# calad0i/da4ml

Measured on AMD Instinct MI355X. Metric: CMVM solves/sec, 256x256 int8 matrix, higher is better.
Workload: dtype u32; 1 GPU; c3_256x256_int8_batch64_single_chain; matrix=256x256 int8 (default_rng(seed).integers(-128,128)), batch_per_gpu=64, parallelism=1 x independent-instance shard, no data-path collective

## Files before the change

### __graft_entry__.py

```python

import subprocess
import sys
from pathlib import Path

ROOT = Path(__file__).resolve().parent
if str(ROOT) not in sys.path:
    sys.path.insert(0, str(ROOT))


def build() -> None:
    subprocess.run(['make', '-C', str(ROOT / 'da4ml_amd' / 'csrc')], check=True)
    subprocess.run(['make', '-C', str(ROOT / 'oracle'), 'liboracle.so', 'ref'], check=True)
    subprocess.run(['make', '-C', str(ROOT / 'tests' / 'model')], check=True)
    subprocess.run(['make', '-C', str(ROOT / 'tests' / 'geometry')], check=True)
    subprocess.run(['make', '-C', str(ROOT / 'tests' / 'tie_order')], check=True)
    subprocess.run(['make', '-C', str(ROOT / 'tests' / 'dc_rank')], check=True)
    subprocess.run(['make', '-C', str(ROOT / 'tests' / 'emu')], check=True)
    import da4ml_amd
    from da4ml_amd import _binary

    lib = _binary.lib()
    missing = [s for s in _binary.EXPORTS if not hasattr(lib, s)]
    assert not missing, f'libda4ml_hip.so lacks {missing}'


def smoke() -> None:
    import numpy as np

    from da4ml_amd import _binary
# ... 16 lines not shown
```

### da4ml_amd/_binary/__init__.py

```python

from __future__ import annotations

import ctypes as C
from pathlib import Path
from types import SimpleNamespace

import numpy as np

from .._marshal import pipeline_from_stages, stage_from_arrays

import os as _os

_LIB_PATH = Path(_os.environ['DA4ML_HIP_LIB']).resolve() if _os.environ.get('DA4ML_HIP_LIB') else Path(__file__).resolve().parent.parent / 'libda4ml_hip.so'
_lib = None

_f32p = np.ctypeslib.ndpointer(np.float32, flags='C_CONTIGUOUS')
_i64p = np.ctypeslib.ndpointer(np.int64, flags='C_CONTIGUOUS')
_i32p = np.ctypeslib.ndpointer(np.int32, flags='C_CONTIGUOUS')

EXPORTS = (
    'da_last_error da_last_error_code da_version da_device_count da_set_device da_get_lsb_loc da_iceil_log2 da_cost_add da_int_arr_to_csd '
    'da_csd_decompose da_kernel_decompose da_solve da_solve_batch da_solve_batch_seeded da_solve_batch_opts da_solve_sharded da_rccl_unique_id da_rccl_shutdown da_solve_sharded_rccl da_comm_abort da_shard_exchanged_elements da_n_stages da_picked da_stage_info da_stage_copy '
    'da_result_stats da_free da_timings da_engine_stats da_dais_run da_dais_last_error da_dais_run_on'
).split()
# ... 425 lines not shown
        _raise(rc)
    return RawBatch([res[i] for i in range(n)])


def timings(reset: bool = False) -> dict:
    t = np.zeros(32, np.float64)
    e = np.zeros(16, np.float64)
    lib().da_engine_stats(e, 16)
    rc = lib().da_timings(t, int(reset))
    if rc != 0:
        _raise(rc)
    names = ('loop_ms', 'dist_ms', 'total_ms', 'lockstep_iters', 'iterations', 'rescans', 'partners', 'chains', 'table_bytes', 'arena_bytes',
             'select_ms_sampled', 'update_ms_sampled', 'samples', 'found', 'inserts', 'cell_reads', 'block_bytes', 'cell_bytes',
             'sel_load_bounds', 'sel_argmax', 'sel_newrow', 'sel_substitute', 'sel_prefix', 'sel_claims', 'sel_special',
             'upd_fetch', 'upd_probe', 'upd_cells', 'upd_blocks', 'upd_create', 'retries', 'sampled_chain_launches')
    extra = ('select_bytes', 'host_launch_ms', 'fast_steps', 'search_bounds', 'search_argmax', 'search_excluded', 'search_steps_timed', 'search_stale_rereads', 'search_touch_rereads', 'search_rounds', 'search_long_lists', 'search_longest_list', 'search_full_passes', 'search_list_entries', 'manycol_chains')
    return {**dict(zip(names, t.tolist())), **dict(zip(extra, e.tolist()))}


_DAIS_EXECUTORS = {'host': 0, 'cpu': 0, 'device': 1, 'gpu': 1, 'host-scalar': 2}


def dais_interp_run(bin_logic, data, n_threads: int = 1, executor: str = 'host'):
    prog = np.ascontiguousarray(np.ravel(bin_logic), dtype=np.int32)
    if prog.size < 4:
        raise RuntimeError('Invalid binary logic data')
    n_in, n_out = int(prog[2]), int(prog[3])
    x = np.ascontiguousarray(np.ravel(data), dtype=np.float64)
    assert n_in > 0 and x.size % n_in == 0, f'Input size {x.size} is not divisible by {n_in}'
    n_samples = x.size // n_in
    out = np.zeros((n_samples, max(n_out, 0)), dtype=np.float64)
# ... 17 lines not shown
```

### da4ml_amd/csrc/cmvm_capi.cc

```cpp

#include <cstdlib>
#include <chrono>
#include <cstdio>
#include <pthread.h>

#include <algorithm>
#include <atomic>
#include <limits>
#include <cstring>
#include <memory>
#include <mutex>
#include <new>
#include <string>
#include <vector>

#include "../../include/da4ml_hip.h"
#include "cmvm_gpu.h"
#include "cmvm_host.h"
#include "cmvm_rccl.h"
#include "cmvm_shard.h"

namespace {

thread_local std::string g_err;
// ... 385 lines not shown
        for (int q = 0; q < 12; ++q) v[18 + q] = g.phase_cycles[q];
        v[30] = (double)g.retries;
        v[31] = g.sampled_chain_launches;
        std::memcpy(t, v, sizeof v);
        if (reset) be.reset_timings();
        return DA_OK;
    } catch (const std::exception &e) {
        return fail(e);
    }
}

int da_engine_stats(double *out, int n) {
    std::lock_guard<LibraryMutex> lk(g_mutex);
    try {
        const da::gpu::GpuTimings &g = backend().timings();
        const double v[16] = {g.select_bytes, g.host_launch_ms, (double)g.fast_steps, g.search_cycles[0], g.search_cycles[1], g.search_cycles[2], g.search_cycles[3], g.search_diag[0], g.search_diag[1], g.search_diag[2], g.search_diag[3], g.search_diag[4], g.search_diag[5], g.search_diag[6], (double)g.manycol_chains, 0.0};
        const int m = n < 16 ? (n < 0 ? 0 : n) : 16;
        for (int i = 0; i < m; ++i) out[i] = v[i];
        return m;
    } catch (const std::exception &e) {
        fail(e);
        return 0;
    }
}

}
```

### da4ml_amd/csrc/cmvm_engine.hip

```cpp

#include <hip/hip_runtime.h>

#include <algorithm>
#include <atomic>
#include <chrono>
#include <cmath>
#include <cstdio>
#include <cstdlib>
#include <cstring>
#include <memory>
#include <mutex>
#include <numeric>
#include <stdexcept>
#include <string>
#include <thread>
#include <type_traits>
#include <vector>

#include "cmvm_core.h"
#include "cmvm_geometry.h"
#include "cmvm_gpu.h"
#include "cmvm_host.h"

namespace da {
// ... 241 lines not shown
    unsigned long long st_sel_bytes;
    unsigned long long st_phase[12];
    SpecPick spec[2];
    unsigned int c_n[2], l_n[2];
    CandEntry c_list[2][CAND_CAP];
    CandEntry l_list[2][TOUCH_CAP];
    uint32_t *sp_cnt;
    unsigned long long st_fast;
    unsigned long long st_qphase[4];
#ifdef DA_STEP_CLOCKS
    unsigned long long clk[2][4];
#endif
    unsigned long long st_qdiag[9];
    unsigned long long tie_seed;
    float dc_weight;
};

__constant__ Log2Table c_log2;

__device__ __forceinline__ int lane_id() { return threadIdx.x & (WAVE - 1); }
__device__ __forceinline__ int wave_id() { return threadIdx.x / WAVE; }

template <int CTRL, int ROW_MASK> __device__ __forceinline__ uint32_t dpp_u32(uint32_t identity, uint32_t v) {
    return (uint32_t)__builtin_amdgcn_update_dpp((int)identity, (int)v, CTRL, ROW_MASK, 0xF, false);
}
constexpr int DPP_ROW_SHR1 = 0x111, DPP_ROW_SHR2 = 0x112, DPP_ROW_SHR4 = 0x114, DPP_ROW_SHR8 = 0x118, DPP_ROW_BCAST15 = 0x142, DPP_ROW_BCAST31 = 0x143;
#define DA_DPP_REDUCE32(v, ident, OP)                                   \
    v = OP(v, dpp_u32<DPP_ROW_SHR1, 0xF>(ident, v));                    \
    v = OP(v, dpp_u32<DPP_ROW_SHR2, 0xF>(ident, v));                    \
    v = OP(v, dpp_u32<DPP_ROW_SHR4, 0xF>(ident, v));                    \
// ... 202 lines not shown
    } else {
        atomicMax(gen(&c.grec[grp].glow), w_old);
    }
}
__device__ __forceinline__ void fold_entry(const Ctx &c, uint32_t rank, unsigned long long tie) {
    if (c.rword && bound_word(rank, tie) >= c.rword) {
        const unsigned int at = atomicAdd(c.cn, 1u);
        if (at < (unsigned int)CAND_CAP) {
            c.cl[at].rank = rank;
            c.cl[at].tie = tie;
        }
    }
}
__device__ __forceinline__ DA_GLOBAL uint8_t *hidx_ptr(const Ctx &c) { return reinterpret_cast<DA_GLOBAL uint8_t *>(c.hrank + ((size_t)c.cmask + 1)); }

template <bool SEEDED, bool WEIGHTED>
__device__ __forceinline__ void publish_new_block(const BlockEval<SEEDED, WEIGHTED> &ev, int slot, uint32_t lo, uint32_t hi, int ov, float dl, unsigned long long best) {
    const Ctx &c = ev.c;
    const uint32_t rank = ev.rank_of_best(best), idx = ev.idx_of_best(best);
    store_hdr(c, slot, ov, dl, rank, idx);
    c.hrank[slot] = rank;
    hidx_ptr(c)[slot] = (uint8_t)idx;
    if (rank) {
        group_note(c, slot, 0ull, bound_word(rank, ev.tie(lo, hi, idx)));
        fold_entry(c, rank, ev.tie(lo, hi, idx));
    }
}

template <bool SEEDED, bool WEIGHTED, class CntFn>
__device__ bool table_insert(const BlockEval<SEEDED, WEIGHTED> &ev, uint32_t lo, uint32_t hi, const RowInfo &ra, const RowInfo &rb, CntFn cnt_of, bool tally = true) {
    const Ctx &c = ev.c;
    int lane = lane_id();
    unsigned long long key = pack_pair(lo, hi);
    int slot = table_claim(c, key, hash_pair(lo, hi));
    if (slot < 0) {
        if (lane == 0) c.g->error = E_TABLE_CAPACITY;
        return false;
// ... 12 lines not shown
    if (lane == 0) {
        publish_new_block(ev, slot, lo, hi, ov, dl, best);
        if (tally) atomicAdd(&c.g->n_live, 1u);
    }
    return true;
}

template <bool SEEDED, bool WEIGHTED>
__device__ __forceinline__ void block_commit(const BlockEval<SEEDED, WEIGHTED> &ev, int slot, unsigned long long key, const BlkHdr &h, unsigned long long best, int alive, bool tally = true) {
    const Ctx &c = ev.c;
    const uint32_t lo = (uint32_t)key, hi = (uint32_t)(key >> 32);
    const unsigned long long w_old = ev.word(lo, hi, h.rank, h.idx);
    if (!alive) {
        c.hrank[slot] = 0;
        c.hkey[slot] = c.tomb;
        if (tally) atomicSub(&c.g->n_live, 1u);
        if (h.rank) group_note(c, slot, w_old, 0ull);
        return;
    }
    const uint32_t rank = ev.rank_of_best(best), idx = ev.idx_of_best(best);
    if (rank != h.rank) c.hrank[slot] = rank;
    if (rank != h.rank || idx != h.idx) store_best(c, slot, rank, idx);
    if (idx != h.idx) hidx_ptr(c)[slot] = (uint8_t)idx;
    if (rank != h.rank || (rank && idx != h.idx)) group_note(c, slot, w_old, ev.word(lo, hi, rank, idx));
    if (rank) fold_entry(c, rank, ev.tie(lo, hi, idx));
}

template <bool SEEDED, bool WEIGHTED, class CntFn>
__device__ bool table_update(const BlockEval<SEEDED, WEIGHTED> &ev, int slot, unsigned long long key, CntFn new_cnt, bool tally = true) {
    const Ctx &c = ev.c;
// ... 108 lines not shown
}

__device__ __forceinline__ void fill16(void *p, size_t bytes, uint32_t v, size_t t0, size_t stride) {
    da_i4 *q = reinterpret_cast<da_i4 *>(p);
    const da_i4 w = da_i4{(int)v, (int)v, (int)v, (int)v};
    for (size_t i = t0, n = (bytes + 15) / 16; i < n; i += stride) q[i] = w;
}
__global__ void __launch_bounds__(256) k_init_state(ChainDev *chains) {
    const ChainDev &ch = chains[blockIdx.y];
    const size_t t0 = (size_t)blockIdx.x * blockDim.x + threadIdx.x, stride = (size_t)gridDim.x * blockDim.x;
    fill16(ch.stamp, sizeof(uint32_t) * (size_t)ch.rcap, 0u, t0, stride);
    fill16(ch.hkey, sizeof(unsigned long long) * (size_t)ch.C, 0xFFFFFFFFu, t0, stride);
    fill16(ch.hrank, sizeof(uint32_t) * (size_t)ch.C, 0u, t0, stride);
    for (size_t i = t0; i < (size_t)ch.n_groups; i += stride) ch.grec[i] = GroupRec{0ull, 0ull, 0ull, 1u, 0u};
    fill16(ch.colbits, sizeof(uint32_t) * (size_t)ch.n_out * ch.cb_words, 0u, t0, stride);
}

template <class Cell> __global__ void __launch_bounds__(256) k_init_cells(ChainDev *chains) {
    using O = CellOps<Cell>;
    using F = RowFmt<Cell>;
    ChainDev &ch = chains[blockIdx.y];
    int j = blockIdx.x * (blockDim.x / WAVE) + wave_id();
    if (j >= ch.n_out) return;
    auto *rl = reinterpret_cast<typename F::Entry *>(ch.rlist);
    int lane = lane_id(), len = 0;
    for (int base = 0; base < ch.n_in; base += WAVE) {
        int i = base + lane;
        Cell c = 0;
        if (i < ch.n_in) {
            bool dead = ch.qints[3 * i] == 0.0f && ch.qints[3 * i + 1] == 0.0f;
// ... 505 lines not shown
    float sp_rb0 = g->spec[par ^ 1].rb.lo, sp_rb1 = g->spec[par ^ 1].rb.hi, sp_rb2 = g->spec[par ^ 1].rb.step, sp_rb3 = g->spec[par ^ 1].rb.lat;
    Ctx c = make_ctx_raw<SEEDED>(g, 2 * iter);
    DA_GLOBAL int *collen = (DA_GLOBAL int *)g->collen;
    DA_GLOBAL da_u2 *rowoff = (DA_GLOBAL da_u2 *)g->rowoff;
    DA_GLOBAL Entry *rl = (DA_GLOBAL Entry *)g->rlist;
    DA_GLOBAL Cell *mA = (DA_GLOBAL Cell *)g->mA, *mB = (DA_GLOBAL Cell *)g->mB;
    DA_GLOBAL int *mcol = (DA_GLOBAL int *)g->mcol;
    DA_GLOBAL unsigned long long *collist = (DA_GLOBAL unsigned long long *)g->collist;
    DA_GLOBAL uint16_t *cmap = (DA_GLOBAL uint16_t *)g->cmap;
    DA_GLOBAL uint32_t *colbits = (DA_GLOBAL uint32_t *)g->colbits;
    DA_GLOBAL uint32_t *pl_ids = (DA_GLOBAL uint32_t *)g->pl_ids;
    DA_GLOBAL unsigned long long *plist = (DA_GLOBAL unsigned long long *)g->plist;
    DA_GLOBAL da_i4 *picks = (DA_GLOBAL da_i4 *)g->picks;
    DA_GLOBAL uint32_t *sp_cnt = (DA_GLOBAL uint32_t *)g->sp_cnt;
    DA_GLOBAL int32_t *cs_slab = (DA_GLOBAL int32_t *)g->cs_slab, *cs_flags = (DA_GLOBAL int32_t *)g->cs_flags;
    pin_sgpr(was_done, had_error, lcap, claim_words, n_rows0, rcap, cbw, adder_size, carry_size, offN, rl_cap, n_live0, live_peak0, step_mant, step_tab, n_step_mant);
    pin_sgpr(sp_word, sp_tie, cn_prev, cl_prev, sp_ax, sp_ay, sp_bx, sp_by, sp_ra0, sp_ra1, sp_ra2, sp_ra3, sp_rb0, sp_rb1, sp_rb2, sp_rb3);
    pin_sgpr(c.n_out, c.n_bits, c.K, c.Kpad, c.rows);
    pin_sgpr(collen, rowoff, rl, mA, mB, mcol, collist, cmap, colbits, pl_ids, plist, picks, sp_cnt);
    if constexpr (SHARDED) pin_sgpr(cs_slab, cs_flags);
    if constexpr (SEEDED) pin_sgpr(c.seed);
    const int n_out = c.n_out, Kpad = c.Kpad, nb = c.n_bits;
    auto shard_stop = [&](int err) {
        if constexpr (SHARDED) {
            const int fw = (n_rows0 + 3) / 4;
            for (int w = threadIdx.x; w < fw; w += SEL2_THREADS) cs_flags[w] = 0;
            if (threadIdx.x == 0) {
                const bool cap = err == E_ROW_CAPACITY || err == E_TABLE_CAPACITY || err == E_LIST_CAPACITY;
                cs_flags[fw] = 1;
                cs_flags[fw + 1] = cap ? 1 : 0;
                cs_flags[fw + 2] = err != E_OK && !cap ? 1 : 0;
            }
        }
    };
    if (was_done) {
        shard_stop(had_error);
// ... 8 lines not shown
    Idx *s_bpos = s_col + n_out;
    int *s_clen = reinterpret_cast<int *>(s_bpos + n_out);
    Idx *s_cm = reinterpret_cast<Idx *>(s_clen + n_out);
    uint32_t *s_or = reinterpret_cast<uint32_t *>(s_cm + n_out);
    if constexpr (MANYCOL) {
        s_bent = nullptr;
        s_clen = nullptr;
        s_cnt = reinterpret_cast<uint32_t *>(smem);
        s_len = reinterpret_cast<int *>(s_cnt + 6 * Kpad);
        s_or = reinterpret_cast<uint32_t *>(s_len + n_out + 1);
        s_col = reinterpret_cast<Idx *>(s_or + claim_words);
        s_bpos = s_col + n_out;
        s_cm = s_bpos + n_out;
    }
    constexpr int NW = SEL2_THREADS / WAVE;
    __shared__ int s_np, s_part[NW];
    __shared__ unsigned int s_matches;
    __shared__ RowInfo s_new;
    __shared__ unsigned long long s_am_tie[NW];
    __shared__ uint32_t s_am_rank[NW];
    constexpr int IDS_LDS = DA_IDS_LDS;
    __shared__ uint32_t s_ids[IDS_LDS];
    __shared__ Log2Table s_log2;

    const int tid = threadIdx.x, lane = lane_id(), wid = wave_id();

    SEL_TIMER_DECL
    SEL_TIMER_MARK(0)
    if (had_error != E_OK) {
        if (tid == 0) {
            g->done = 1;
// ... 11 lines not shown
    da_u2 refA = da_u2{sp_ax, sp_ay}, refB = da_u2{sp_bx, sp_by};
    RowInfo ra = RowInfo{sp_ra0, sp_ra1, sp_ra2, sp_ra3}, rb = RowInfo{sp_rb0, sp_rb1, sp_rb2, sp_rb3};
    if (fast && !from_spec) {
        refA = rowoff[A];
        refB = rowoff[B];
        ra = load_row(c.rows, A);
        rb = load_row(c.rows, B);
    }
    {
        int clen0 = 0;
        if constexpr (!MANYCOL) clen0 = collen[tid < n_out ? tid : 0];
        const bool want_log2 = (adder_size >= 0 || carry_size >= 0) && tid < (int)(sizeof(Log2Table) / 4);
        const uint32_t l2w = want_log2 ? reinterpret_cast<const uint32_t *>(&c_log2)[tid] : 0u;
        if (tid == 0) {
            s_np = 0;
            s_matches = 0;
            g->c_n[par] = 0;
        }
        if (tid < n_out) {
            if constexpr (!MANYCOL) s_clen[tid] = clen0;
            s_cm[tid] = 0;
            s_bpos[tid] = 0;
        }
        if (want_log2) reinterpret_cast<uint32_t *>(&s_log2)[tid] = l2w;
        for (int w = tid; w < claim_words; w += SEL2_THREADS) s_or[w] = 0;
        for (int j = tid + SEL2_THREADS; j < n_out; j += SEL2_THREADS) {
            if constexpr (!MANYCOL) s_clen[j] = collen[j];
            s_cm[j] = 0;
            s_bpos[j] = 0;
        }
// ... 41 lines not shown
        shard_stop(E_LIST_CAPACITY);
        return 1;
    }
    DA_GLOBAL Entry *rlA = rl + refA.x, *rlB = rl + refB.x, *rlN = rl + offN;
    Entry eA0 = rl[tid < lenA ? refA.x + (uint32_t)tid : 0u], eB0 = rl[tid < lenB ? refB.x + (uint32_t)tid : 0u];
    load_fence();
    RowInfo rn = RowInfo{0.0f, 0.0f, 0.0f, 0.0f};
    int derr = 0;
    if (tid == 0) {
        qint_add_pair(ra, rb, shift, sub, rn.lo, rn.hi, rn.step);
        float dlat = adder_dlat(ra, rb, shift, sub, adder_size, carry_size, s_log2, StepLog2{n_step_mant, step_mant, step_tab}, derr);
        rn.lat = (ra.lat < rb.lat ? rb.lat : ra.lat) + dlat;
        s_new = rn;
    }
    for (int k = tid; k < 6 * Kpad; k += SEL2_THREADS) s_cnt[k] = 0;
    if (tid >= lenA) eA0 = F::none();
    if (same || tid >= lenB) eB0 = F::none();
    pin_vgpr(eA0, eB0);
    if (!same) {
        if (tid < lenB) {
            if constexpr (!MANYCOL) s_bent[tid] = eB0;
            s_bpos[F::col(eB0)] = (Idx)(tid + 1);
        }
        for (int t = tid + SEL2_THREADS; t < lenB; t += SEL2_THREADS) {
            const Entry e = rlB[t];
            if constexpr (!MANYCOL) s_bent[t] = e;
            s_bpos[F::col(e)] = (Idx)(t + 1);
        }
    }
    if (tid == 0) {
// ... 105 lines not shown
    __syncthreads();
    SEL_TIMER_MARK(4)
    SEL_TIMER_MARK(5)
    if constexpr (SHARDED) {
        for (int k = tid; k < 6 * c.K; k += SEL2_THREADS) {
            const int sp = k / c.K;
            cs_slab[k] = (same && (sp == 1 || sp == 2 || sp == 4)) ? 0 : (int32_t)s_cnt[sp * Kpad + (k - sp * c.K)];
        }
    } else
        for (int k = tid; k < 6 * Kpad; k += SEL2_THREADS) sp_cnt[k] = s_cnt[k];
    {
        const DA_GLOBAL uint32_t *cb = colbits;
        const int nwords = (int)((Nw + 31) >> 5), chunks = (nwords + WAVE - 1) / WAVE;
        DA_GLOBAL uint32_t *ids = pl_ids;
        const bool split = chunks * 4 <= NW && m >= 8 && nwords <= claim_words;
        if (split) {
            const int c = wid % chunks, part = wid / chunks, ways = (NW - c + chunks - 1) / chunks;
            const int w = c * WAVE + lane;
            if (w < nwords) {
                uint32_t bits = 0;
                for (int k = part; k < m; k += ways) bits |= cb[(size_t)s_col[k] * cbw + w];
                if (bits) atomicOr(&s_or[w], bits);
            }
            __syncthreads();
        }
        for (int wb = wid * WAVE; wb < nwords; wb += SEL2_THREADS) {
            const int w = wb + lane;
            uint32_t bits = 0;
            if (w < nwords) {
                if (split)
                    bits = s_or[w];
                else
                    for (int k = 0; k < m; ++k) bits |= cb[(size_t)s_col[k] * cbw + w];
                if ((int)(A >> 5) == w) bits &= ~(1u << (A & 31));
                if ((int)(B >> 5) == w) bits &= ~(1u << (B & 31));
                if ((int)(Nw >> 5) == w) bits &= ~(1u << (Nw & 31));
            }
            if constexpr (SHARDED) {
                const int fw = (int)((Nw + 3) / 4);
                if (w < nwords) {
#pragma unroll
                    for (int q = 0; q < 8; ++q) {
                        const uint32_t b = (bits >> (4 * q)) & 0xFu;
                        if (8 * w + q < fw) cs_flags[8 * w + q] = (int32_t)((b & 1u) | ((b & 2u) << 7) | ((b & 4u) << 14) | ((b & 8u) << 21));
                    }
                }
                continue;
            }
            const int cnt = popc32(bits), inc = (int)wave_scan_add_u32((uint32_t)cnt);
            const int wave_total = __builtin_amdgcn_readlane(inc, WAVE - 1);
            if (wave_total == 0) continue;
            int base = 0;
            if (lane == 0) base = atomicAdd(&s_np, wave_total);
            int at = __builtin_amdgcn_readfirstlane(base) + inc - cnt;
            while (bits) {
                const uint32_t id = (uint32_t)(w << 5) + (uint32_t)ctz32(bits);
                if (at < IDS_LDS)
                    s_ids[at] = id;
                else
                    ids[at] = id;
                ++at;
                bits &= bits - 1;
            }
        }
    }
    SEL_TIMER_MARK(6)
    __syncthreads();
    if constexpr (SHARDED) {
        if (tid < SHARD_TRAILER) cs_flags[(int)((Nw + 3) / 4) + tid] = 0;
    }
    {
        const int np = s_np;
        const DA_GLOBAL uint32_t *ids = pl_ids;
        for (int t = tid; t < np; t += 2 * SEL2_THREADS) {
            const int t2 = t + SEL2_THREADS;
            const bool has2 = t2 < np;
            const uint32_t r1 = t < IDS_LDS ? s_ids[t] : ids[t];
            const uint32_t r2 = !has2 ? r1 : t2 < IDS_LDS ? s_ids[t2] : ids[t2];
            const da_u2 ro1 = rowoff[r1], ro2 = rowoff[r2];
            load_fence();
            plist[t] = ref_pack(r1, ro1.y, ro1.x);
            if (has2) plist[t2] = ref_pack(r2, ro2.y, ro2.x);
        }
    }
    SEL_TIMER_MARK(7)
    if (tid == 0) {
        SEL_TIMER_FLUSH
        rowoff[Nw] = da_u2{offN, (uint32_t)m};
        g->rl_used = offN + (uint32_t)m;
        g->m = m;
        g->n_partners = s_np;
        atomicAdd(&g->st_matches, (unsigned long long)s_matches);
        atomicAdd(&g->st_partners, (unsigned long long)s_np);
        atomicAdd(&g->st_cells, (unsigned long long)s_np * (unsigned)m);
        if (fast) atomicAdd(&g->st_fast, 1ull);
        {
            const unsigned long long eb = sizeof(Entry), cb = sizeof(Cell);
            const unsigned long long nwords = (Nw + 31) >> 5;
            atomicAdd(&g->st_sel_bytes, 4ull * (unsigned)n_out + 64ull + 2ull * eb * (unsigned)(lenA + (same ? 0 : lenB)) + 4ull * (unsigned)m * nwords + 20ull * (unsigned)s_np +
                                            (unsigned)m * (4ull + 2ull * cb + eb + 8ull + 12ull) + 2ull * (unsigned)n_out + 6ull * 4ull * (unsigned)Kpad);
        }
        g->A = A;
        g->B = B;
        g->Nw = Nw;
        g->pk_shift = shift;
        g->pk_sub = sub;
        g->n_rows = (int)Nw + 1;
        g->iter = iter + 1;
    }
    return 0;
}
#ifndef DA_SEL2_WAVES
#define DA_SEL2_WAVES 4
#endif
// ... 797 lines not shown
```

### da4ml_amd/csrc/cmvm_geometry.h

```cpp
#pragma once

#include <algorithm>
#include <cstdint>

#include "cmvm_core.h"
#include "cmvm_host.h"

namespace da {

constexpr int TABLE_HEURISTIC_LOG2 = 25;
constexpr int TABLE_MAX_LOG2 = 30;
constexpr int TABLE_SLOTS_PER_PAIR = 2;

struct TableGeometry {
    uint32_t C;
    int gs_log2;
    int n_groups;
    long long rcap;
};

inline uint64_t pow2_ceil_u64(uint64_t v) {
    uint64_t p = 1;
    while (p < v && p < (1ull << 62)) p <<= 1;
    return p;
}

inline TableGeometry table_geometry(const ChainJob &job, long long prep_pairs, long long prep_digits, double table_scale, double row_scale,
// ... 32 lines not shown
```

### da4ml_amd/csrc/cmvm_gpu.h

```cpp
#pragma once

#include <memory>

#include "cmvm_host.h"
#include "cmvm_shard.h"

namespace da {
namespace gpu {

struct GpuTimings {
    double loop_ms = 0;
    double dist_ms = 0;
    double total_ms = 0;
    long long lockstep_iters = 0;
    long long iterations = 0;
    long long rescans = 0;
    long long partners = 0;
    long long chains = 0;
    long long retries = 0;
    long long dist_calls = 0;
    double select_ms_sampled = 0, update_ms_sampled = 0;
    long long samples = 0;
    long long manycol_chains = 0;
    double sampled_chain_launches = 0;
    long long found = 0, inserts = 0, cell_reads = 0;
    double key_bytes = 0;
    double cell_bytes = 0;
    double phase_cycles[12] = {0};
    double table_bytes = 0;
    double arena_bytes = 0;
    double select_bytes = 0;
    double host_launch_ms = 0;
// ... 32 lines not shown
```

### da4ml_amd/csrc/hip_batch.h

```cpp
#pragma once
#ifndef DA_ENGINE_TU
#error "hip_batch.h is a part of cmvm_engine.hip"
#endif

struct HipBackend::Impl::Batch {
    Impl &im;
    const ChainJob *const jobs;
    ChainOut *const outs;
    const int n;
    const hipStream_t st;
    Batch(Impl &impl, const ChainJob *j, ChainOut *o, int count) : im(impl), jobs(j), outs(o), n(count), st(impl.stream) {}

    std::vector<ChainDev> desc, sorted, fin;
    std::vector<StepLog2Host> step_tabs;
    std::vector<GatherPiece> pieces;

    ChainDev *d_desc = nullptr;
    int max_n_out = 0;
    std::vector<Geometry> geo;
    std::vector<size_t> a_off;
    size_t arena_bytes = 0, budget = 0, free_b = 0;
    std::vector<int> order;
    std::vector<char> manycol;
    static constexpr int N_VAR = 16;
// ... 37 lines not shown
        hipLaunchKernelGGL(k_prepare, dim3(n), dim3(256), (size_t)max_n_out * 4, st, d_desc);
        HIP_CHECK(hipGetLastError());
        HIP_CHECK(hipMemcpyAsync(desc.data(), d_desc, sizeof(ChainDev) * (size_t)n, hipMemcpyDeviceToHost, st));
        HIP_CHECK(hipStreamSynchronize(st));
    }

    void plan(double row_scale) {
        static const GeometryErrors msg{"kernel needs more than 30 CSD digits per entry (the reference overflows int32 there); unsupported",
                                        "problem too large for the row-reference format (rows < 2^24, columns < 4096, list entries < 2^28)"};
        step_tabs.resize(n);
        for (int i = 0; i < n; ++i)
            if (jobs[i].adder_size >= 0 || jobs[i].carry_size >= 0) step_tabs[i].build(jobs[i].qints, jobs[i].n_in);
        geo.resize(n);
        a_off.resize(n);
        for (int i = 0; i < n; ++i) {
            geo[i] = derive_geometry(desc[i], jobs[i], jobs[i].n_out, (int)step_tabs[i].mant.size(), im.table_scale, row_scale, msg);
            ChainDev tmp;
            a_off[i] = arena_bytes;
            arena_bytes += carve_chain(nullptr, jobs[i].n_out, geo[i], tmp);
        }
        size_t total_b = 0;
        HIP_CHECK(hipMemGetInfo(&free_b, &total_b));
        budget = (size_t)(0.85 * (double)(free_b + im.arena.cap));
        if (const char *e = std::getenv("DA4ML_HIP_MEM_BUDGET_MB")) budget = (size_t)std::atoll(e) << 20;
    }

    void init_chains() {
        unsigned char *arena = static_cast<unsigned char *>(im.arena.get(arena_bytes));
        manycol.resize(n);
        for (int i = 0; i < n; ++i) {
            carve_chain(arena + a_off[i], jobs[i].n_out, geo[i], desc[i]);
            manycol[i] = sel2_manycol(im.device, jobs[i].n_out, geo[i], im.manycol_from);
            apply_geometry(desc[i], geo[i], sel2_lds_budget(im.device, geo[i].wide, manycol[i]), manycol[i]);
            desc[i].done = (jobs[i].method == M_DUMMY || jobs[i].method < 0) ? 1 : 0;
        }
        for (int i = 0; i < n; ++i) upload_step_table(desc[i], step_tabs[i], st);
        HIP_CHECK(hipMemcpyAsync(d_desc, desc.data(), sizeof(ChainDev) * (size_t)n, hipMemcpyHostToDevice, st));
        HIP_CHECK(hipMemsetAsync(im.d_done, 0, sizeof(unsigned int), st));
        hipLaunchKernelGGL(k_init_state, dim3(128, n), dim3(256), 0, st, d_desc);
        HIP_CHECK(hipGetLastError());

        order.resize(n);
        std::iota(order.begin(), order.end(), 0);
        std::stable_sort(order.begin(), order.end(), [&](int a, int b) { return variant(a) < variant(b); });
        bool permuted = false;
        for (int i = 0; i < n; ++i) permuted |= order[i] != i;
        if (permuted) {
            sorted.resize(n);
// ... 298 lines not shown
            const ChainDev &d = fin[s];
            for (int q = 0; q < 12; ++q) tm.phase_cycles[q] += (double)d.st_phase[q];
            for (int q = 0; q < 4; ++q) tm.search_cycles[q] += (double)d.st_qphase[q];
            tm.search_diag[0] += (double)d.st_qdiag[0], tm.search_diag[1] += (double)d.st_qdiag[1], tm.search_diag[2] += (double)d.st_qdiag[4];
            tm.search_diag[3] += (double)d.st_qdiag[5], tm.search_diag[4] = std::max(tm.search_diag[4], (double)d.st_qdiag[6]), tm.search_diag[5] += (double)d.st_qdiag[7], tm.search_diag[6] += (double)d.st_qdiag[8];
            tm.fast_steps += (long long)d.st_fast;
            tm.found += (long long)d.st_found;
            tm.inserts += (long long)d.st_inserts;
            tm.cell_reads += (long long)d.st_cells;
            tm.key_bytes += 2.0 * d.K * (double)(d.st_found + d.st_inserts);
            tm.cell_bytes += (geo[order[s]].wide ? 8.0 : 4.0) * (double)d.st_cells;
            tm.iterations += d.iter;
            tm.rescans += (long long)d.st_rescans;
            tm.select_bytes += (double)d.st_sel_bytes + 32.0 * (double)d.n_groups * (double)d.iter + (double)d.st_rescans * ((double)(4u << d.gs_log2) + 24.0);
            tm.partners += (long long)d.st_partners;
            tm.table_bytes += (double)d.C * (8.0 + 4.0 + (double)(1 << d.pb_log2));
        }
        tm.loop_ms += loop_ms;
        tm.host_launch_ms += host_launch_ms;
        tm.lockstep_iters += launched_iters;
        tm.chains += n;
        for (int i = 0; i < n; ++i) tm.manycol_chains += manycol[i] ? 1 : 0;
        tm.arena_bytes = std::max(tm.arena_bytes, (double)arena_bytes);
    }
};

void HipBackend::run_chains(const ChainJob *jobs, ChainOut *outs, int n) {
    if (n <= 0) return;
    Impl &im = *impl_;
    HIP_CHECK(hipSetDevice(im.device));
// ... 49 lines not shown
```

### da4ml_amd/csrc/hip_chain_setup.h

```cpp
#pragma once
#ifndef DA_ENGINE_TU
#error "hip_chain_setup.h is a part of cmvm_engine.hip"
#endif

struct HipBackend::Impl {
    int device = 0;
    PinnedBuffer pinned, pinned_up;
    hipStream_t stream = nullptr;
    static constexpr int MAX_LANES = 8;
    hipStream_t lanes[MAX_LANES] = {nullptr, nullptr, nullptr, nullptr, nullptr, nullptr, nullptr, nullptr};
    int launch_threads = 2;
    int n_lanes = 4;
    int upd_total_blocks = 2560;
    DeviceBuffer arena, desc_buf, io_buf, gather_buf, piece_buf;
    unsigned int *d_done = nullptr;
    unsigned int *h_done = nullptr;
    hipStream_t poll_stream = nullptr;
    GpuTimings timings;
    double table_scale = 1.0;
    int manycol_from = 0;
    struct Batch;
};

HipBackend::HipBackend(int device) : impl_(new Impl) {
    impl_->device = device;
    HIP_CHECK(hipSetDevice(device));
    HIP_CHECK(hipStreamCreateWithFlags(&impl_->stream, hipStreamNonBlocking));
    impl_->lanes[0] = impl_->stream;
    for (int l = 1; l < Impl::MAX_LANES; ++l) HIP_CHECK(hipStreamCreateWithFlags(&impl_->lanes[l], hipStreamNonBlocking));
    if (const char *e = std::getenv("DA4ML_HIP_TABLE_SCALE")) impl_->table_scale = std::max(1e-4, std::atof(e));
    if (const char *e = std::getenv("DA4ML_HIP_MANYCOL_FROM")) impl_->manycol_from = std::max(0, std::atoi(e));
    if (const char *e = std::getenv("DA4ML_HIP_ROW_SCALE")) row_scale_ = std::max(1e-4, std::atof(e));
    if (const char *e = std::getenv("DA4ML_HIP_UPD_BLOCKS")) impl_->upd_total_blocks = std::max(2, std::atoi(e));
    if (const char *e = std::getenv("DA4ML_HIP_LAUNCH_THREADS")) impl_->launch_threads = std::max(1, std::atoi(e));
    if (const char *e = std::getenv("DA4ML_HIP_LANES")) impl_->n_lanes = std::max(1, std::min((int)Impl::MAX_LANES, std::atoi(e)));
    HIP_CHECK(hipMalloc(&impl_->d_done, sizeof(unsigned int)));
    HIP_CHECK(hipHostMalloc(&impl_->h_done, 2 * sizeof(unsigned int), hipHostMallocDefault));
    HIP_CHECK(hipStreamCreateWithFlags(&impl_->poll_stream, hipStreamNonBlocking));
    Log2Table t = measure_log2_table();
    HIP_CHECK(hipMemcpyToSymbol(HIP_SYMBOL(c_log2), &t, sizeof t));
}
HipBackend::~HipBackend() {
    (void)hipSetDevice(impl_->device);
    if (impl_->d_done) (void)hipFree(impl_->d_done);
    if (impl_->h_done) (void)hipHostFree(impl_->h_done);
// ... 1 lines not shown
    if (impl_->stream) (void)hipStreamDestroy(impl_->stream);
    for (int l = 1; l < Impl::MAX_LANES; ++l)
        if (impl_->lanes[l]) (void)hipStreamDestroy(impl_->lanes[l]);
}
const GpuTimings &HipBackend::timings() const { return impl_->timings; }
void HipBackend::reset_timings() { impl_->timings = GpuTimings{}; }
void *HipBackend::stream() const { return impl_->stream; }

namespace {

struct Geometry {
    bool wide;
    int n_mant = 0;
    int n_bits, K, Kpad, rcap, lcap, gs_log2, n_groups, pk_cap, pb_log2;
    uint32_t C, rl_cap;
};

template <class F> void with_sel2(bool wide, bool manycol, bool seeded, F &&f) {
    with_cell(wide, [&](auto c) { with_flag(manycol, [&](auto mc) { with_flag(seeded, [&](auto sd) { f(c, mc, sd); }); }); });
}
template <bool SHARDED> void sel2_allow_lds(bool wide, size_t bytes, bool manycol = false, bool seeded = false) {
    if constexpr (SHARDED)
        with_cell(wide, [&](auto c) {
            HIP_CHECK(hipFuncSetAttribute(reinterpret_cast<const void *>(&k_iter_select2<decltype(c), true>), hipFuncAttributeMaxDynamicSharedMemorySize, (int)bytes));
        });
    else
        with_sel2(wide, manycol, seeded, [&](auto c, auto mc, auto sd) {
            HIP_CHECK(hipFuncSetAttribute(reinterpret_cast<const void *>(&k_iter_select2<decltype(c), false, decltype(mc)::value, decltype(sd)::value>), hipFuncAttributeMaxDynamicSharedMemorySize, (int)bytes));
        });
}
// ... 79 lines not shown
        HIP_CHECK(hipFuncSetAttribute(reinterpret_cast<const void *>(&k_iter_update<decltype(c), true, true>), hipFuncAttributeMaxDynamicSharedMemorySize, (int)bytes));
        HIP_CHECK(hipFuncSetAttribute(reinterpret_cast<const void *>(&k_iter_update<decltype(c), false, false, true>), hipFuncAttributeMaxDynamicSharedMemorySize, (int)bytes));
        HIP_CHECK(hipFuncSetAttribute(reinterpret_cast<const void *>(&k_iter_update<decltype(c), true, false, true>), hipFuncAttributeMaxDynamicSharedMemorySize, (int)bytes));
        HIP_CHECK(hipFuncSetAttribute(reinterpret_cast<const void *>(&k_iter_update<decltype(c), false, true, true>), hipFuncAttributeMaxDynamicSharedMemorySize, (int)bytes));
        HIP_CHECK(hipFuncSetAttribute(reinterpret_cast<const void *>(&k_iter_update<decltype(c), true, true, true>), hipFuncAttributeMaxDynamicSharedMemorySize, (int)bytes));
    });
}
int claim_words_for(int n_out, const Geometry &g, size_t budget, bool manycol = false) {
    const size_t words = ((size_t)g.rcap + 31) / 32, fixed = align_up(sel2_fixed_lds(n_out, g, manycol), 16);
    return words * 4 <= 64 * 1024 && fixed + words * 4 + 16 <= budget ? (int)words : 0;
}

struct GeometryErrors {
    const char *digits, *row_ref;
};
Geometry derive_geometry(const ChainDev &d, const ChainJob &job, int n_loc, int n_mant, double table_scale, double row_scale, const GeometryErrors &msg) {
    Geometry g;
    g.n_bits = d.prep_nbits;
    if (g.n_bits > 30) throw std::runtime_error(msg.digits);
    g.wide = g.n_bits > 12 || n_loc > 256;
    g.n_mant = n_mant;
    g.K = key_count(g.n_bits);
    g.Kpad = (g.K + 3) & ~3;
    g.pb_log2 = 5;
    while ((1 << g.pb_log2) < 16 + 2 * g.Kpad) ++g.pb_log2;
    const long long D0 = d.prep_digits;
    const TableGeometry tg = table_geometry(job, d.prep_pairs, D0, table_scale, row_scale, MAX_GROUPS);
    g.rcap = tg.rcap < (1 << REF_ROW_BITS) ? (int)tg.rcap : (1 << REF_ROW_BITS);
    g.lcap = job.n_in + d.prep_maxdcol + 1;
    g.pk_cap = (int)std::min<long long>(D0 + 1, (long long)1 << 30);
    const long long rl_want = (long long)job.n_in * n_loc + D0 + n_loc + 64;
    if (rl_want >= (1ll << REF_OFF_BITS) || g.rcap >= (1 << REF_ROW_BITS) || n_loc >= (1 << REF_LEN_BITS)) throw std::runtime_error(msg.row_ref);
    g.rl_cap = (uint32_t)rl_want;
    g.C = tg.C;
    g.gs_log2 = tg.gs_log2;
    g.n_groups = tg.n_groups;
    return g;
}

size_t carve_chain(unsigned char *base, int n_loc, const Geometry &g, ChainDev &d) {
    Carver c(base);
    size_t cell = g.wide ? 8 : 4, entry = g.wide ? 16 : 4;
    size_t n_out = n_loc;
    d.rlist = c.take<unsigned char>((size_t)g.rl_cap * entry);
    d.rowoff = c.take<da_u2>(g.rcap);
    d.rows = c.take<RowInfo>(g.rcap);
    d.stamp = c.take<uint32_t>(g.rcap);
    d.collist = c.take<unsigned long long>(n_out * (size_t)g.lcap);
    d.collen = c.take<int>(n_out);
    d.hkey = c.take<unsigned long long>(g.C);
    d.hrank = c.take<uint32_t>((size_t)g.C + ((size_t)g.C + 3) / 4);
// ... 6 lines not shown
    d.mA = c.take<unsigned char>(n_out * cell);
    d.mB = c.take<unsigned char>(n_out * cell);
    d.plist = c.take<unsigned long long>(g.rcap);
    d.sp_cnt = c.take<uint32_t>((size_t)6 * g.Kpad);
    d.picks = c.take<int4>(g.rcap);
    d.fin_row = c.take<uint32_t>(n_out * (size_t)g.lcap);
    d.fin_cell = c.take<unsigned long long>(n_out * (size_t)g.lcap);
    d.fin_count = c.take<uint32_t>(n_out);
    d.fin_start = c.take<uint32_t>(n_out + 1);
    d.pk_cap = g.pk_cap;
    d.pk_row = c.take<uint32_t>((size_t)g.pk_cap);
    d.pk_cell = c.take<unsigned long long>((size_t)g.pk_cap);
    d.pk_lat = c.take<float>(g.rcap);
    d.step_mant = c.take<uint32_t>((size_t)std::max(g.n_mant, 1));
    d.step_tab = c.take<float>((size_t)std::max(g.n_mant, 1) * 256);
    return align_up(c.off, 256);
}

void apply_geometry(ChainDev &d, const Geometry &g, size_t lds_budget, bool manycol = false) {
    d.n_bits = g.n_bits;
    d.K = g.K;
    d.Kpad = g.Kpad;
    d.rcap = g.rcap;
    d.lcap = g.lcap;
    d.gs_log2 = g.gs_log2;
    d.n_groups = g.n_groups;
    d.C = g.C;
    d.cmask = g.C - 1;
    d.pb_log2 = g.pb_log2;
    d.rl_cap = g.rl_cap;
    d.rl_used = (uint32_t)d.n_in * (uint32_t)d.n_out;
    d.n_rows = d.n_in;
    d.claim_words = claim_words_for(d.n_out, g, lds_budget, manycol);
    d.iter = 0;
    d.cb_words = (g.rcap + 31) / 32;
    d.n_step_mant = g.n_mant;
}
void upload_step_table(const ChainDev &d, const StepLog2Host &t, hipStream_t st) {
    if (!d.n_step_mant) return;
    HIP_CHECK(hipMemcpyAsync(const_cast<uint32_t *>(d.step_mant), t.mant.data(), t.mant.size() * 4, hipMemcpyHostToDevice, st));
    HIP_CHECK(hipMemcpyAsync(const_cast<float *>(d.step_tab), t.tab.data(), t.tab.size() * 4, hipMemcpyHostToDevice, st));
}

void fill_result(ChainOut &o, const ChainDev &d) {
    o = ChainOut{};
    o.error = d.error;
    o.unknown_method_hit = d.unknown_hit != 0;
    o.n_bits = d.n_bits;
    o.stats.iterations = d.iter;
    o.stats.digits0 = d.prep_digits;
// ... 8 lines not shown
```

Before: 115.1 solves/s.

## Filter selection partners with a pair-existence bitmap to skip known pairs

Adds a per-chain row-by-row bitmap recording which row pairs already have a live hash-table block. Blocks set the bits when published and clear them when they die, and rows reset their bits when reused. During partner selection, candidate rows whose pair with A or B is already present are masked out, so fewer partners are handed to the update stage. In exchange it adds global atomics on every block publish and clear, extra bitmap reads and arena memory (capped by a budget), and an env switch to disable it; it is off in the sharded path.

```diff
diff --git a/__graft_entry__.py b/__graft_entry__.py
--- a/__graft_entry__.py
+++ b/__graft_entry__.py
@@ -13,6 +13,7 @@
     subprocess.run(['make', '-C', str(ROOT / 'oracle'), 'liboracle.so', 'ref'], check=True)
     subprocess.run(['make', '-C', str(ROOT / 'tests' / 'model')], check=True)
     subprocess.run(['make', '-C', str(ROOT / 'tests' / 'geometry')], check=True)
+    subprocess.run(['make', '-C', str(ROOT / 'tests' / 'pair_bits')], check=True)
     subprocess.run(['make', '-C', str(ROOT / 'tests' / 'tie_order')], check=True)
     subprocess.run(['make', '-C', str(ROOT / 'tests' / 'dc_rank')], check=True)
     subprocess.run(['make', '-C', str(ROOT / 'tests' / 'emu')], check=True)
diff --git a/da4ml_amd/_binary/__init__.py b/da4ml_amd/_binary/__init__.py
--- a/da4ml_amd/_binary/__init__.py
+++ b/da4ml_amd/_binary/__init__.py
@@ -463,7 +463,7 @@
              'select_ms_sampled', 'update_ms_sampled', 'samples', 'found', 'inserts', 'cell_reads', 'block_bytes', 'cell_bytes',
              'sel_load_bounds', 'sel_argmax', 'sel_newrow', 'sel_substitute', 'sel_prefix', 'sel_claims', 'sel_special',
              'upd_fetch', 'upd_probe', 'upd_cells', 'upd_blocks', 'upd_create', 'retries', 'sampled_chain_launches')
-    extra = ('select_bytes', 'host_launch_ms', 'fast_steps', 'search_bounds', 'search_argmax', 'search_excluded', 'search_steps_timed', 'search_stale_rereads', 'search_touch_rereads', 'search_rounds', 'search_long_lists', 'search_longest_list', 'search_full_passes', 'search_list_entries', 'manycol_chains')
+    extra = ('select_bytes', 'host_launch_ms', 'fast_steps', 'search_bounds', 'search_argmax', 'search_excluded', 'search_steps_timed', 'search_stale_rereads', 'search_touch_rereads', 'search_rounds', 'search_long_lists', 'search_longest_list', 'search_full_passes', 'search_list_entries', 'manycol_chains', 'partners_handed')
     return {**dict(zip(names, t.tolist())), **dict(zip(extra, e.tolist()))}
 
 
diff --git a/da4ml_amd/csrc/cmvm_capi.cc b/da4ml_amd/csrc/cmvm_capi.cc
--- a/da4ml_amd/csrc/cmvm_capi.cc
+++ b/da4ml_amd/csrc/cmvm_capi.cc
@@ -423,7 +423,7 @@
     std::lock_guard<LibraryMutex> lk(g_mutex);
     try {
         const da::gpu::GpuTimings &g = backend().timings();
-        const double v[16] = {g.select_bytes, g.host_launch_ms, (double)g.fast_steps, g.search_cycles[0], g.search_cycles[1], g.search_cycles[2], g.search_cycles[3], g.search_diag[0], g.search_diag[1], g.search_diag[2], g.search_diag[3], g.search_diag[4], g.search_diag[5], g.search_diag[6], (double)g.manycol_chains, 0.0};
+        const double v[16] = {g.select_bytes, g.host_launch_ms, (double)g.fast_steps, g.search_cycles[0], g.search_cycles[1], g.search_cycles[2], g.search_cycles[3], g.search_diag[0], g.search_diag[1], g.search_diag[2], g.search_diag[3], g.search_diag[4], g.search_diag[5], g.search_diag[6], (double)g.manycol_chains, (double)g.partners_handed};
         const int m = n < 16 ? (n < 0 ? 0 : n) : 16;
         for (int i = 0; i < m; ++i) out[i] = v[i];
         return m;
diff --git a/da4ml_amd/csrc/cmvm_engine.hip b/da4ml_amd/csrc/cmvm_engine.hip
--- a/da4ml_amd/csrc/cmvm_engine.hip
+++ b/da4ml_amd/csrc/cmvm_engine.hip
@@ -279,6 +279,10 @@
     unsigned long long st_qdiag[9];
     unsigned long long tie_seed;
     float dc_weight;
+    uint32_t *pairbits;
+    int pair_rows, pair_stride;
+    int pair_filter;
+    unsigned long long st_handed;
 };
 
 __constant__ Log2Table c_log2;
@@ -511,6 +515,21 @@
 }
 __device__ __forceinline__ DA_GLOBAL uint8_t *hidx_ptr(const Ctx &c) { return reinterpret_cast<DA_GLOBAL uint8_t *>(c.hrank + ((size_t)c.cmask + 1)); }
 
+__device__ __forceinline__ void pair_bits_set(const Ctx &c, uint32_t lo, uint32_t hi) {
+    DA_GLOBAL uint32_t *pb = (DA_GLOBAL uint32_t *)c.g->pairbits;
+    const uint32_t pbw = (uint32_t)c.g->pair_stride, prows = (uint32_t)c.g->pair_rows;
+    if (!pb || hi >= prows) return;
+    atomicOr(gen(&pb[lo * pbw + (hi >> 5)]), 1u << (hi & 31));
+    if (lo != hi) atomicOr(gen(&pb[hi * pbw + (lo >> 5)]), 1u << (lo & 31));
+}
+__device__ __forceinline__ void pair_bits_clear(const Ctx &c, uint32_t lo, uint32_t hi) {
+    DA_GLOBAL uint32_t *pb = (DA_GLOBAL uint32_t *)c.g->pairbits;
+    const uint32_t pbw = (uint32_t)c.g->pair_stride, prows = (uint32_t)c.g->pair_rows;
+    if (!pb || hi >= prows) return;
+    atomicAnd(gen(&pb[lo * pbw + (hi >> 5)]), ~(1u << (hi & 31)));
+    if (lo != hi) atomicAnd(gen(&pb[hi * pbw + (lo >> 5)]), ~(1u << (lo & 31)));
+}
+
 template <bool SEEDED, bool WEIGHTED>
 __device__ __forceinline__ void publish_new_block(const BlockEval<SEEDED, WEIGHTED> &ev, int slot, uint32_t lo, uint32_t hi, int ov, float dl, unsigned long long best) {
     const Ctx &c = ev.c;
@@ -518,6 +537,7 @@
     store_hdr(c, slot, ov, dl, rank, idx);
     c.hrank[slot] = rank;
     hidx_ptr(c)[slot] = (uint8_t)idx;
+    pair_bits_set(c, lo, hi);
     if (rank) {
         group_note(c, slot, 0ull, bound_word(rank, ev.tie(lo, hi, idx)));
         fold_entry(c, rank, ev.tie(lo, hi, idx));
@@ -560,6 +580,7 @@
     if (!alive) {
         c.hrank[slot] = 0;
         c.hkey[slot] = c.tomb;
+        pair_bits_clear(c, lo, hi);
         if (tally) atomicSub(&c.g->n_live, 1u);
         if (h.rank) group_note(c, slot, w_old, 0ull);
         return;
@@ -698,6 +719,7 @@
     fill16(ch.hrank, sizeof(uint32_t) * (size_t)ch.C, 0u, t0, stride);
     for (size_t i = t0; i < (size_t)ch.n_groups; i += stride) ch.grec[i] = GroupRec{0ull, 0ull, 0ull, 1u, 0u};
     fill16(ch.colbits, sizeof(uint32_t) * (size_t)ch.n_out * ch.cb_words, 0u, t0, stride);
+    if (ch.pairbits) fill16(ch.pairbits, sizeof(uint32_t) * (size_t)min(ch.n_in, ch.pair_rows) * ch.pair_stride, 0u, t0, stride);
 }
 
 template <class Cell> __global__ void __launch_bounds__(256) k_init_cells(ChainDev *chains) {
@@ -1233,12 +1255,19 @@
     DA_GLOBAL da_i4 *picks = (DA_GLOBAL da_i4 *)g->picks;
     DA_GLOBAL uint32_t *sp_cnt = (DA_GLOBAL uint32_t *)g->sp_cnt;
     DA_GLOBAL int32_t *cs_slab = (DA_GLOBAL int32_t *)g->cs_slab, *cs_flags = (DA_GLOBAL int32_t *)g->cs_flags;
+    DA_GLOBAL uint32_t *pairbits = (DA_GLOBAL uint32_t *)g->pairbits;
+    int pair_filter = g->pair_filter, pair_rows = g->pair_rows, pair_stride = g->pair_stride;
     pin_sgpr(was_done, had_error, lcap, claim_words, n_rows0, rcap, cbw, adder_size, carry_size, offN, rl_cap, n_live0, live_peak0, step_mant, step_tab, n_step_mant);
     pin_sgpr(sp_word, sp_tie, cn_prev, cl_prev, sp_ax, sp_ay, sp_bx, sp_by, sp_ra0, sp_ra1, sp_ra2, sp_ra3, sp_rb0, sp_rb1, sp_rb2, sp_rb3);
     pin_sgpr(c.n_out, c.n_bits, c.K, c.Kpad, c.rows);
     pin_sgpr(collen, rowoff, rl, mA, mB, mcol, collist, cmap, colbits, pl_ids, plist, picks, sp_cnt);
     if constexpr (SHARDED) pin_sgpr(cs_slab, cs_flags);
     if constexpr (SEEDED) pin_sgpr(c.seed);
+    if constexpr (SHARDED)
+        pairbits = nullptr;
+    else
+        pin_sgpr(pairbits, pair_filter, pair_rows, pair_stride);
+    const bool filtering = pairbits && pair_filter;
     const int n_out = c.n_out, Kpad = c.Kpad, nb = c.n_bits;
     auto shard_stop = [&](int err) {
         if constexpr (SHARDED) {
@@ -1277,7 +1306,7 @@
         s_cm = s_bpos + n_out;
     }
     constexpr int NW = SEL2_THREADS / WAVE;
-    __shared__ int s_np, s_part[NW];
+    __shared__ int s_np, s_np_all, s_part[NW];
     __shared__ unsigned int s_matches;
     __shared__ RowInfo s_new;
     __shared__ unsigned long long s_am_tie[NW];
@@ -1319,6 +1348,7 @@
         const uint32_t l2w = want_log2 ? reinterpret_cast<const uint32_t *>(&c_log2)[tid] : 0u;
         if (tid == 0) {
             s_np = 0;
+            s_np_all = 0;
             s_matches = 0;
             g->c_n[par] = 0;
         }
@@ -1390,6 +1420,10 @@
         s_new = rn;
     }
     for (int k = tid; k < 6 * Kpad; k += SEL2_THREADS) s_cnt[k] = 0;
+    if constexpr (!SHARDED) {
+        if (pairbits && (int)Nw < pair_rows)
+            for (int w = tid; w < pair_stride; w += SEL2_THREADS) pairbits[Nw * (uint32_t)pair_stride + (uint32_t)w] = 0u;
+    }
     if (tid >= lenA) eA0 = F::none();
     if (same || tid >= lenB) eB0 = F::none();
     pin_vgpr(eA0, eB0);
@@ -1525,24 +1559,33 @@
         const int nwords = (int)((Nw + 31) >> 5), chunks = (nwords + WAVE - 1) / WAVE;
         DA_GLOBAL uint32_t *ids = pl_ids;
         const bool split = chunks * 4 <= NW && m >= 8 && nwords <= claim_words;
+        uint32_t filt = ~0u;
+        auto filter_word = [&](int w) -> uint32_t {
+            if ((int)A >= pair_rows || (int)B >= pair_rows || w >= pair_stride) return ~0u;
+            return pairbits[A * (uint32_t)pair_stride + (uint32_t)w] | pairbits[B * (uint32_t)pair_stride + (uint32_t)w];
+        };
         if (split) {
             const int c = wid % chunks, part = wid / chunks, ways = (NW - c + chunks - 1) / chunks;
             const int w = c * WAVE + lane;
             if (w < nwords) {
+                if (filtering && part == 0) filt = filter_word(w);
                 uint32_t bits = 0;
                 for (int k = part; k < m; k += ways) bits |= cb[(size_t)s_col[k] * cbw + w];
                 if (bits) atomicOr(&s_or[w], bits);
             }
             __syncthreads();
         }
+        int n_all = 0;
         for (int wb = wid * WAVE; wb < nwords; wb += SEL2_THREADS) {
             const int w = wb + lane;
             uint32_t bits = 0;
             if (w < nwords) {
                 if (split)
                     bits = s_or[w];
-                else
+                else {
+                    if (filtering) filt = filter_word(w);
                     for (int k = 0; k < m; ++k) bits |= cb[(size_t)s_col[k] * cbw + w];
+                }
                 if ((int)(A >> 5) == w) bits &= ~(1u << (A & 31));
                 if ((int)(B >> 5) == w) bits &= ~(1u << (B & 31));
                 if ((int)(Nw >> 5) == w) bits &= ~(1u << (Nw & 31));
@@ -1558,6 +1601,8 @@
                 }
                 continue;
             }
+            n_all += popc32(bits);
+            bits &= filt;
             const int cnt = popc32(bits), inc = (int)wave_scan_add_u32((uint32_t)cnt);
             const int wave_total = __builtin_amdgcn_readlane(inc, WAVE - 1);
             if (wave_total == 0) continue;
@@ -1574,6 +1619,13 @@
                 bits &= bits - 1;
             }
         }
+        if constexpr (!SHARDED) {
+            if (filtering) {
+                n_all = (int)wave_scan_add_u32((uint32_t)n_all);
+                const int wave_all = __builtin_amdgcn_readlane(n_all, WAVE - 1);
+                if (lane == 0 && wave_all) atomicAdd(&s_np_all, wave_all);
+            }
+        }
     }
     SEL_TIMER_MARK(6)
     __syncthreads();
@@ -1602,13 +1654,15 @@
         g->m = m;
         g->n_partners = s_np;
         atomicAdd(&g->st_matches, (unsigned long long)s_matches);
-        atomicAdd(&g->st_partners, (unsigned long long)s_np);
-        atomicAdd(&g->st_cells, (unsigned long long)s_np * (unsigned)m);
+        const int np_all = filtering ? s_np_all : s_np;
+        atomicAdd(&g->st_partners, (unsigned long long)np_all);
+        atomicAdd(&g->st_cells, (unsigned long long)np_all * (unsigned)m);
+        atomicAdd(&g->st_handed, (unsigned long long)s_np);
         if (fast) atomicAdd(&g->st_fast, 1ull);
         {
             const unsigned long long eb = sizeof(Entry), cb = sizeof(Cell);
             const unsigned long long nwords = (Nw + 31) >> 5;
-            atomicAdd(&g->st_sel_bytes, 4ull * (unsigned)n_out + 64ull + 2ull * eb * (unsigned)(lenA + (same ? 0 : lenB)) + 4ull * (unsigned)m * nwords + 20ull * (unsigned)s_np +
+            atomicAdd(&g->st_sel_bytes, 4ull * (unsigned)n_out + 64ull + 2ull * eb * (unsigned)(lenA + (same ? 0 : lenB)) + 4ull * (unsigned)m * nwords + 20ull * (unsigned)np_all +
                                             (unsigned)m * (4ull + 2ull * cb + eb + 8ull + 12ull) + 2ull * (unsigned)n_out + 6ull * 4ull * (unsigned)Kpad);
         }
         g->A = A;
diff --git a/da4ml_amd/csrc/cmvm_geometry.h b/da4ml_amd/csrc/cmvm_geometry.h
--- a/da4ml_amd/csrc/cmvm_geometry.h
+++ b/da4ml_amd/csrc/cmvm_geometry.h
@@ -11,6 +11,20 @@
 constexpr int TABLE_HEURISTIC_LOG2 = 25;
 constexpr int TABLE_MAX_LOG2 = 30;
 constexpr int TABLE_SLOTS_PER_PAIR = 2;
+
+constexpr uint64_t PAIR_BITS_BUDGET = 64ull << 20;
+inline long long pair_bits_rows(long long rcap, uint64_t budget_bytes) {
+    if (rcap <= 0) return 0;
+    const uint64_t max_words = (1ull << 32) - 1;
+    uint64_t r = 0;
+    for (uint64_t step = 1ull << 20; step >= 32; step >>= 1) {
+        const uint64_t words = (r + step) * ((r + step) / 32);
+        if (words <= budget_bytes / 4 && words <= max_words) r += step;
+    }
+    const uint64_t rows = (uint64_t)rcap, full = rows * ((rows + 31) / 32);
+    return (long long)(full <= budget_bytes / 4 && full <= max_words ? rows : std::min(r, rows / 32 * 32));
+}
+inline uint64_t pair_bits_stride(long long rows) { return ((uint64_t)rows + 31) / 32; }
 
 struct TableGeometry {
     uint32_t C;
diff --git a/da4ml_amd/csrc/cmvm_gpu.h b/da4ml_amd/csrc/cmvm_gpu.h
--- a/da4ml_amd/csrc/cmvm_gpu.h
+++ b/da4ml_amd/csrc/cmvm_gpu.h
@@ -16,6 +16,7 @@
     long long iterations = 0;
     long long rescans = 0;
     long long partners = 0;
+    long long partners_handed = 0;
     long long chains = 0;
     long long retries = 0;
     long long dist_calls = 0;
diff --git a/da4ml_amd/csrc/hip_batch.h b/da4ml_amd/csrc/hip_batch.h
--- a/da4ml_amd/csrc/hip_batch.h
+++ b/da4ml_amd/csrc/hip_batch.h
@@ -75,7 +75,7 @@
         geo.resize(n);
         a_off.resize(n);
         for (int i = 0; i < n; ++i) {
-            geo[i] = derive_geometry(desc[i], jobs[i], jobs[i].n_out, (int)step_tabs[i].mant.size(), im.table_scale, row_scale, msg);
+            geo[i] = derive_geometry(desc[i], jobs[i], jobs[i].n_out, (int)step_tabs[i].mant.size(), im.table_scale, row_scale, msg, im.pair_bits_budget);
             ChainDev tmp;
             a_off[i] = arena_bytes;
             arena_bytes += carve_chain(nullptr, jobs[i].n_out, geo[i], tmp);
@@ -89,10 +89,13 @@
     void init_chains() {
         unsigned char *arena = static_cast<unsigned char *>(im.arena.get(arena_bytes));
         manycol.resize(n);
+        const char *filter_env = std::getenv("DA4ML_HIP_PAIR_FILTER");
+        const int pair_filter = !(filter_env && std::atoi(filter_env) == 0);
         for (int i = 0; i < n; ++i) {
             carve_chain(arena + a_off[i], jobs[i].n_out, geo[i], desc[i]);
             manycol[i] = sel2_manycol(im.device, jobs[i].n_out, geo[i], im.manycol_from);
             apply_geometry(desc[i], geo[i], sel2_lds_budget(im.device, geo[i].wide, manycol[i]), manycol[i]);
+            desc[i].pair_filter = pair_filter;
             desc[i].done = (jobs[i].method == M_DUMMY || jobs[i].method < 0) ? 1 : 0;
         }
         for (int i = 0; i < n; ++i) upload_step_table(desc[i], step_tabs[i], st);
@@ -421,6 +424,7 @@
             tm.rescans += (long long)d.st_rescans;
             tm.select_bytes += (double)d.st_sel_bytes + 32.0 * (double)d.n_groups * (double)d.iter + (double)d.st_rescans * ((double)(4u << d.gs_log2) + 24.0);
             tm.partners += (long long)d.st_partners;
+            tm.partners_handed += (long long)d.st_handed;
             tm.table_bytes += (double)d.C * (8.0 + 4.0 + (double)(1 << d.pb_log2));
         }
         tm.loop_ms += loop_ms;
diff --git a/da4ml_amd/csrc/hip_chain_setup.h b/da4ml_amd/csrc/hip_chain_setup.h
--- a/da4ml_amd/csrc/hip_chain_setup.h
+++ b/da4ml_amd/csrc/hip_chain_setup.h
@@ -18,6 +18,7 @@
     hipStream_t poll_stream = nullptr;
     GpuTimings timings;
     double table_scale = 1.0;
+    uint64_t pair_bits_budget = PAIR_BITS_BUDGET;
     int manycol_from = 0;
     struct Batch;
 };
@@ -29,6 +30,7 @@
     impl_->lanes[0] = impl_->stream;
     for (int l = 1; l < Impl::MAX_LANES; ++l) HIP_CHECK(hipStreamCreateWithFlags(&impl_->lanes[l], hipStreamNonBlocking));
     if (const char *e = std::getenv("DA4ML_HIP_TABLE_SCALE")) impl_->table_scale = std::max(1e-4, std::atof(e));
+    if (const char *e = std::getenv("DA4ML_HIP_PAIR_BITS_MB")) impl_->pair_bits_budget = (uint64_t)std::max(0.0, std::atof(e) * 1048576.0);
     if (const char *e = std::getenv("DA4ML_HIP_MANYCOL_FROM")) impl_->manycol_from = std::max(0, std::atoi(e));
     if (const char *e = std::getenv("DA4ML_HIP_ROW_SCALE")) row_scale_ = std::max(1e-4, std::atof(e));
     if (const char *e = std::getenv("DA4ML_HIP_UPD_BLOCKS")) impl_->upd_total_blocks = std::max(2, std::atoi(e));
@@ -60,6 +62,7 @@
     int n_mant = 0;
     int n_bits, K, Kpad, rcap, lcap, gs_log2, n_groups, pk_cap, pb_log2;
     uint32_t C, rl_cap;
+    int pair_rows = 0;
 };
 
 template <class F> void with_sel2(bool wide, bool manycol, bool seeded, F &&f) {
@@ -169,7 +172,8 @@
 struct GeometryErrors {
     const char *digits, *row_ref;
 };
-Geometry derive_geometry(const ChainDev &d, const ChainJob &job, int n_loc, int n_mant, double table_scale, double row_scale, const GeometryErrors &msg) {
+Geometry derive_geometry(const ChainDev &d, const ChainJob &job, int n_loc, int n_mant, double table_scale, double row_scale, const GeometryErrors &msg,
+                         uint64_t pair_bits_budget = 0) {
     Geometry g;
     g.n_bits = d.prep_nbits;
     if (g.n_bits > 30) throw std::runtime_error(msg.digits);
@@ -190,6 +194,7 @@
     g.C = tg.C;
     g.gs_log2 = tg.gs_log2;
     g.n_groups = tg.n_groups;
+    g.pair_rows = (int)pair_bits_rows(g.rcap, pair_bits_budget);
     return g;
 }
 
@@ -226,6 +231,7 @@
     d.pk_lat = c.take<float>(g.rcap);
     d.step_mant = c.take<uint32_t>((size_t)std::max(g.n_mant, 1));
     d.step_tab = c.take<float>((size_t)std::max(g.n_mant, 1) * 256);
+    d.pairbits = g.pair_rows ? c.take<uint32_t>((size_t)g.pair_rows * pair_bits_stride(g.pair_rows)) : nullptr;
     return align_up(c.off, 256);
 }
 
@@ -246,6 +252,8 @@
     d.claim_words = claim_words_for(d.n_out, g, lds_budget, manycol);
     d.iter = 0;
     d.cb_words = (g.rcap + 31) / 32;
+    d.pair_rows = g.pair_rows;
+    d.pair_stride = (int)pair_bits_stride(g.pair_rows);
     d.n_step_mant = g.n_mant;
 }
 void upload_step_table(const ChainDev &d, const StepLog2Host &t, hipStream_t st) {
```

Result: slower. 113.6 solves/s (-1.3%).
